# jkulhanek/viewformer

Measured on NVIDIA H100. Metric: novel views/sec (128x128, 9-ctx), higher is better.
Workload: dtype f32 encoder (bit-exact codes) + bf16 transformer/decoder

## Files before the change

### viewformer_b200/csrc/vf_tc_gemm.cu

```cuda
#include "vf_wgmma.cuh"
#include <stdlib.h>

namespace {
using namespace vftc;

constexpr int BLOCK_M = 128;
constexpr int ROW_BYTES = 128;
constexpr int A_STAGE_BYTES = BLOCK_M * ROW_BYTES;
constexpr int NUM_EPI_WARPS = 8;
constexpr int NUM_MMA_THREADS = 32 * NUM_EPI_WARPS;
constexpr int NUM_THREADS = NUM_MMA_THREADS + 128;

struct TcParams {
    CUtensorMap tmA, tmB;
    int conv;
    int M, Ncols;
    int num_k_blocks;
    int batch2;
    int tiles_m, tiles_n, total_tiles;
    int a_bm1, a_bm2, b_bm1, b_bm2;
    int TW, TH, TN, tiles_x, tiles_y, OH, OW, Nimg, cin_blocks, bk_elems;
    int tap_dy[9], tap_dx[9], tap_coff[9];
    int gemm_koff;
    int causal_block, causal_skip_n;
    float alpha;
    const float* bias;
    int bias_mode, act;
    const float* residual;
    float* C_f32;
    __nv_bfloat16* C_bf16;
    long long ldc, c_sb1, c_sb2;
    int vec_ok;
    int halo;
    double* gn_sums;
    int gn_groups, gn_cpg, gn_rows_per_img;
    int exact;
    int exact_kc;
    int exact_clog;
    int exact_kpp;
    int exact_lo_b;
    const float2* norm_mr;
    const float* norm_gamma;
    const float* norm_beta;
    int norm_groups, norm_cpg, norm_swish;
};

constexpr float EXACT_LO_SCALE = 1.0f / 2048.0f;

struct TileInfo {
    int m0, n0, b1, b2, img0, oy0, ox0, nkb;
    bool skip;
};

__device__ __forceinline__ TileInfo decode_tile(const TcParams& p, int t, int block_n) {
    TileInfo ti;
    const int n_tile = t % p.tiles_n;
    const int r = t / p.tiles_n;
    const int m_tile = r % p.tiles_m;
    const int bz = r / p.tiles_m;
    ti.b1 = bz / p.batch2;
    ti.b2 = bz % p.batch2;
    ti.m0 = m_tile * BLOCK_M;
    ti.n0 = n_tile * block_n;
    ti.nkb = p.num_k_blocks;
    ti.skip = false;
    if (p.causal_block > 0) {
        const int lim = ((ti.m0 + BLOCK_M - 1) / p.causal_block + 1) * p.causal_block;
        if (p.causal_skip_n) {
            ti.skip = ti.n0 >= lim;
        } else {
            const int kb = (lim + p.bk_elems - 1) / p.bk_elems;
            if (kb < ti.nkb) ti.nkb = kb;
        }
    }
    ti.img0 = ti.oy0 = ti.ox0 = 0;
    if (p.conv) {
        const int tx = m_tile % p.tiles_x;
        const int q = m_tile / p.tiles_x;
        ti.img0 = (q / p.tiles_y) * p.TN;
        ti.oy0 = (q % p.tiles_y) * p.TH;
        ti.ox0 = tx * p.TW;
    }
    return ti;
}

constexpr int HALO_BYTES = 23552;
__host__ __device__ constexpr int halo_buffers(bool exact) { return exact ? 4 : 2; }
__host__ __device__ constexpr int halo_slots(bool exact) { return exact ? 4 : 6; }
__host__ __device__ constexpr int operand_bytes(int stages, int stage_bytes, int b_stage_bytes, bool exact) {
    return stages * stage_bytes > halo_buffers(exact) * HALO_BYTES + halo_slots(exact) * b_stage_bytes
               ? stages * stage_bytes
               : halo_buffers(exact) * HALO_BYTES + halo_slots(exact) * b_stage_bytes;
}
constexpr int MAX_STAGES = 8;
template <int kBlockN, int kStages, bool kExact>
__host__ __device__ constexpr int tc_smem_bytes() {
    return operand_bytes(kStages, A_STAGE_BYTES + kBlockN * ROW_BYTES, kBlockN * ROW_BYTES, kExact) +
           NUM_EPI_WARPS * 32 * (kBlockN / 2 + 4) * 4  + 1024  + 8 * (2 * MAX_STAGES + 8) ;
}

__device__ __forceinline__ void prefetch_residual_l2(const TcParams& p, const TileInfo& ti, int block_n) {
    const int tw = min(p.TW, p.OW - ti.ox0);
    const uint32_t bytes = (uint32_t)(((long long)(tw - 1) * p.ldc + block_n) * 4);
    for (int r = 0; r < p.TN * p.TH; ++r) {
        const int img = ti.img0 + r / p.TH, oy = ti.oy0 + r % p.TH;
        if (img >= p.Nimg || oy >= p.OH) continue;
        const float* src = p.residual + ((long long)(img * p.OH + oy) * p.OW + ti.ox0) * p.ldc + ti.n0;
        asm volatile("cp.async.bulk.prefetch.L2.global [%0], %1;" ::"l"(src), "r"(bytes) : "memory");
    }
}

__device__ __forceinline__ void normalise_halo(const TcParams& p, uint8_t* tile, int cb, int img, int oy0, int ox0, int tid) {
    const int rows = (p.TW + 2) * (p.TH + 2);
    for (int idx = tid; idx < rows * 8; idx += NUM_MMA_THREADS) {
        const int r = idx >> 3, pc = idx & 7;
        const int py = r / (p.TW + 2), px = r - py * (p.TW + 2);
        const int iy = oy0 - 1 + py, ix = ox0 - 1 + px;
        if (iy < 0 || iy >= p.OH || ix < 0 || ix >= p.OW) continue;
        const int c0 = cb * 64 + ((pc ^ (r & 7)) << 3);
        uint4* ptr = reinterpret_cast<uint4*>(tile + r * ROW_BYTES + pc * 16);
        const uint4 v = *ptr;
        uint32_t w[4] = {v.x, v.y, v.z, v.w};
#pragma unroll
        for (int k = 0; k < 4; ++k) {
            const int c = c0 + 2 * k;
            const float2 ma = __ldg(p.norm_mr + (img * p.norm_groups + c / p.norm_cpg));
            const float2 mb = __ldg(p.norm_mr + (img * p.norm_groups + (c + 1) / p.norm_cpg));
            const float sa = ma.y * __ldg(p.norm_gamma + c), sb = mb.y * __ldg(p.norm_gamma + c + 1);
            float a = __uint_as_float(w[k] << 16), b = __uint_as_float(w[k] & 0xffff0000u);
            a = fmaf(a, sa, __ldg(p.norm_beta + c) - ma.x * sa);
            b = fmaf(b, sb, __ldg(p.norm_beta + c + 1) - mb.x * sb);
            if (p.norm_swish == 1) {
                a = __fdividef(a, 1.0f + __expf(-a));
                b = __fdividef(b, 1.0f + __expf(-b));
            }
            __nv_bfloat162 o = __floats2bfloat162_rn(a, b);
            w[k] = *reinterpret_cast<uint32_t*>(&o);
            if (p.norm_swish == 2) {
                uint32_t h, th;
                asm("mul.rn.bf16x2 %0, %1, %2;" : "=r"(h) : "r"(w[k]), "r"(0x3f003f00u));
                asm("tanh.approx.bf16x2 %0, %1;" : "=r"(th) : "r"(h));
                asm("fma.rn.bf16x2 %0, %1, %2, %1;" : "=r"(w[k]) : "r"(h), "r"(th));
            }
        }
        *ptr = make_uint4(w[0], w[1], w[2], w[3]);
    }
}

template <int kBlockN, int kStages, WgKind kKind>
__global__ void __launch_bounds__(NUM_THREADS, 1) tc_gemm_kernel(const __grid_constant__ TcParams p) {
    constexpr int B_STAGE_BYTES = kBlockN * ROW_BYTES;
    constexpr int STAGE_BYTES = A_STAGE_BYTES + B_STAGE_BYTES;
    constexpr int K_STEPS = 4;
    constexpr int HALF_N = kBlockN / 2;
    constexpr int STG_LD = HALF_N + 4;
    constexpr int STG_BYTES = NUM_EPI_WARPS * 32 * STG_LD * 4;
    constexpr int NACC = kBlockN / 2;
    constexpr bool kExact = kKind == F16;

    extern __shared__ uint8_t smem_raw[];
    uint8_t* smem = reinterpret_cast<uint8_t*>((reinterpret_cast<uintptr_t>(smem_raw) + 1023) & ~(uintptr_t)1023);
    constexpr int OPER_BYTES = operand_bytes(kStages, STAGE_BYTES, B_STAGE_BYTES, kExact);
    float* staging = reinterpret_cast<float*>(smem + OPER_BYTES);
    uint64_t* full_bar = reinterpret_cast<uint64_t*>(smem + OPER_BYTES + STG_BYTES);
    uint64_t* empty_bar = full_bar + MAX_STAGES;
    constexpr int NHB = halo_buffers(kExact);
    uint64_t* a_full_bar = empty_bar + MAX_STAGES;
    uint64_t* a_empty_bar = a_full_bar + NHB;
    constexpr int NG = kStages;
    constexpr int NGH = halo_slots(kExact);
    uint8_t* halo_b_base = smem + NHB * HALO_BYTES;

    const int warp = threadIdx.x >> 5;
    const int lane = threadIdx.x & 31;

    if (threadIdx.x == 0) {
        prefetch_tmap(&p.tmA);
        prefetch_tmap(&p.tmB);
        for (int s = 0; s < MAX_STAGES; ++s) {
            mbar_init(&full_bar[s], 1);
            mbar_init(&empty_bar[s], NUM_MMA_THREADS);
        }
        for (int a = 0; a < NHB; ++a) {
            mbar_init(&a_full_bar[a], 1);
            mbar_init(&a_empty_bar[a], NUM_MMA_THREADS);
        }
        mbar_fence_init();
    }
    __syncthreads();

    if (warp >= NUM_EPI_WARPS) {
        setmaxnreg_dec<40>();
        if (warp == NUM_EPI_WARPS && elect_one()) {
            int stage = 0;
            uint32_t phase = 0;
            int ab = 0;
            uint32_t aphase = 0, tpar = 0;
            for (int t = blockIdx.x; t < p.total_tiles; t += gridDim.x, tpar ^= 1) {
                const TileInfo ti = decode_tile(p, t, kBlockN);
                if (ti.skip) continue;
                const uint32_t halo_bytes = (uint32_t)((p.TW + 2) * (p.TH + 2)) * ROW_BYTES;
                if (kExact && p.halo) {
                    auto load_halves = [&](int h) {
                        for (int cb = 0; cb < p.cin_blocks; ++cb) {
                            const int hb = 2 * h + cb;
                            mbar_wait(&a_empty_bar[hb], tpar ^ 1, "vf_tc_gemm producer(halo)");
                            mbar_expect_tx(&a_full_bar[hb], halo_bytes);
                            tma_load_4d(smem + hb * HALO_BYTES, &p.tmA, &a_full_bar[hb], (h ? 0 : p.exact_clog) + cb * p.bk_elems,
                                        ti.ox0 - 1, ti.oy0 - 1, ti.img0);
                        }
                    };
                    load_halves(0);
                    if (p.residual && p.vec_ok && ti.n0 + kBlockN <= p.Ncols) prefetch_residual_l2(p, ti, kBlockN);
                    int j = 0, tap = 0, cb = 0;
                    for (int kb = 0; kb < ti.nkb; ++kb) {
                        if (kb == NGH) load_halves(1);
                        mbar_wait(&empty_bar[stage], phase ^ 1, "vf_tc_gemm producer");
                        mbar_expect_tx(&full_bar[stage], (uint32_t)B_STAGE_BYTES);
                        tma_load_4d(halo_b_base + stage * B_STAGE_BYTES, &p.tmB, &full_bar[stage],
                                    ((tap * 2 + (j == 1 ? 1 : 0)) * p.cin_blocks + cb) * p.bk_elems, ti.n0, 0, 0);
                        if (++cb == p.cin_blocks) { cb = 0; if (++tap == 9) { tap = 0; ++j; } }
                        if (++stage == NGH) { stage = 0; phase ^= 1; }
                    }
                    continue;
                }
                if (p.halo) {
                    const int nkb = 9 * p.cin_blocks;
                    int tap = 0, cb = 0;
                    for (int kb = 0; kb < nkb; ++kb) {
                        mbar_wait(&empty_bar[stage], phase ^ 1, "vf_tc_gemm producer");
                        mbar_expect_tx(&full_bar[stage], (uint32_t)B_STAGE_BYTES);
                        if (tap == 0) {
                            mbar_wait(&a_empty_bar[ab], aphase ^ 1, "vf_tc_gemm producer(halo)");
                            mbar_expect_tx(&a_full_bar[ab], halo_bytes);
                            tma_load_4d(smem + ab * HALO_BYTES, &p.tmA, &a_full_bar[ab], cb * p.bk_elems, ti.ox0 - 1, ti.oy0 - 1, ti.img0);
                            if (++ab == 2) { ab = 0; aphase ^= 1; }
                        }
                        tma_load_4d(halo_b_base + stage * B_STAGE_BYTES, &p.tmB, &full_bar[stage], (tap * p.cin_blocks + cb) * p.bk_elems,
                                    ti.n0, 0, 0);
                        if (++tap == 9) { tap = 0; ++cb; }
                        if (++stage == NGH) { stage = 0; phase ^= 1; }
                    }
                    continue;
                }
                if (kExact && p.conv && p.residual && p.vec_ok && ti.n0 + kBlockN <= p.Ncols) prefetch_residual_l2(p, ti, kBlockN);
                for (int kb = 0; kb < ti.nkb; ++kb) {
                    mbar_wait(&empty_bar[stage], phase ^ 1, "vf_tc_gemm producer");
                    mbar_expect_tx(&full_bar[stage], (uint32_t)STAGE_BYTES);
                    uint8_t* sa = smem + stage * STAGE_BYTES;
                    uint8_t* sb = sa + A_STAGE_BYTES;
                    int kcoord_b = kb * p.bk_elems;
                    if (p.conv) {
                        int kbr = kb, a_half = 0;
                        if (p.exact) {
                            const int j = kb / p.exact_kpp;
                            kbr = kb - j * p.exact_kpp;
                            a_half = (j == 0) ? p.exact_clog : 0;
                            const int tap_ = kbr / p.cin_blocks, cb_ = kbr - tap_ * p.cin_blocks;
                            kcoord_b = ((tap_ * 2 + (j == 1 ? 1 : 0)) * p.cin_blocks + cb_) * p.bk_elems;
                        }
                        const int tap = kbr / p.cin_blocks;
                        const int cb = kbr - tap * p.cin_blocks;
                        tma_load_4d(sa, &p.tmA, &full_bar[stage], a_half + p.tap_coff[tap] + cb * p.bk_elems, ti.ox0 + p.tap_dx[tap],
                                    ti.oy0 + p.tap_dy[tap], ti.img0);
                    } else {
                        int kcoord_a = kb * p.bk_elems;
                        if (p.exact) {
                            const int j = kb / p.exact_kpp, kbr = kb - j * p.exact_kpp;
                            kcoord_a = (j == 0 ? p.exact_clog : 0) + kbr * p.bk_elems;
                            kcoord_b = (j == 1 ? p.exact_lo_b : 0) + kbr * p.bk_elems;
                        }
                        if (p.gemm_koff) kcoord_a += p.tap_coff[ti.b1];
                        tma_load_4d(sa, &p.tmA, &full_bar[stage], kcoord_a, ti.m0, ti.b2 * p.a_bm2, ti.b1 * p.a_bm1);
                    }
                    tma_load_4d(sb, &p.tmB, &full_bar[stage], kcoord_b, ti.n0, ti.b2 * p.b_bm2, ti.b1 * p.b_bm1);
                    if (++stage == NG) { stage = 0; phase ^= 1; }
                }
            }
        }
        return;
    }

    setmaxnreg_inc<232>();
    const int wg = warp >> 2;
    const int quarter = warp & 3;
    const int col_half = warp >> 2;
    float* stg = staging + warp * (32 * STG_LD);
    int stage = 0, ab = 0;
    uint32_t phase = 0, aphase = 0, tpar = 0;

    const bool col_split = kExact && p.halo && p.TW == 16;
    auto to_staging = [&](const float (&v)[NACC], float sc) {
        const int r_lo = 64 * wg + 16 * (warp & 3) + (lane >> 2);
#pragma unroll
        for (int j = 0; j < NACC / 4; ++j) {
#pragma unroll
            for (int h = 0; h < 2; ++h) {
                const int r = col_split ? 16 * (2 * (warp & 3) + h) + 8 * wg + (lane >> 2) : r_lo + 8 * h;
                const int c = 8 * j + 2 * (lane & 3);
                float* dst = staging + ((c / HALF_N) * 4 + (r >> 5)) * (32 * STG_LD) + (r & 31) * STG_LD + (c % HALF_N);
                *reinterpret_cast<float2*>(dst) = make_float2(v[4 * j + 2 * h] * sc, v[4 * j + 2 * h + 1] * sc);
            }
        }
    };

    for (int t = blockIdx.x; t < p.total_tiles; t += gridDim.x, tpar ^= 1) {
        const TileInfo ti = decode_tile(p, t, kBlockN);
        if (ti.skip) continue;

        float acc[NACC];
        float csum[kExact ? NACC : 1];
        auto k_loop = [&]() {
            const int nkb = (p.halo && !kExact) ? 9 * p.cin_blocks : ti.nkb;
            const int nsmall = p.exact ? 2 * p.exact_kpp / p.exact_kc : 0;
            int prev_stage = -1, prev_halo = -1, in_chunk = 0, ck = 0, tap = 0, j = 0, cb = 0;
            bool fresh = true;
            uint32_t a_base = 0;
            const uint32_t pitch = (uint32_t)(p.TW + 2);
            const uint32_t wg_rows = p.TW == 16 ? 8u : 8u * pitch;
            auto retire_prev = [&]() {
                if (prev_stage >= 0) mbar_arrive(&empty_bar[prev_stage]);
                if (prev_halo >= 0) mbar_arrive(&a_empty_bar[prev_halo]);
                prev_stage = prev_halo = -1;
            };
#pragma unroll 1
            for (int kb = 0; kb < nkb; ++kb) {
                uint64_t adesc, bdesc;
                int this_halo = (p.halo && tap == 8) ? ab : -1;
                if (kExact && p.halo) {
                    const int hb = (j == 0 ? 0 : 2) + cb;
                    if (tap == 0 && j < 2) mbar_wait(&a_full_bar[hb], tpar, "vf_tc_gemm mma(halo)");
                    this_halo = (tap == 8 && j != 1) ? hb : -1;
                    mbar_wait(&full_bar[stage], phase, "vf_tc_gemm mma");
                    const uint32_t a_addr = smem_u32(smem + hb * HALO_BYTES) +
                                            ((uint32_t)(tap / 3) * pitch + (uint32_t)(tap % 3) + (uint32_t)wg * wg_rows) * ROW_BYTES;
                    adesc = sw128_desc(a_addr, pitch * ROW_BYTES);
                    bdesc = sw128_desc(smem_u32(halo_b_base + stage * B_STAGE_BYTES));
                } else if (p.halo) {
                    if (tap == 0) {
                        mbar_wait(&a_full_bar[ab], aphase, "vf_tc_gemm mma(halo)");
                        a_base = smem_u32(smem + ab * HALO_BYTES);
                        if (!kExact && p.norm_mr) {
                            normalise_halo(p, smem + ab * HALO_BYTES, kb / 9, ti.img0, ti.oy0, ti.ox0, threadIdx.x);
                            fence_async_smem();
                            named_sync(1, NUM_MMA_THREADS);
                        }
                    }
                    mbar_wait(&full_bar[stage], phase, "vf_tc_gemm mma");
                    const uint32_t a_addr = a_base + ((uint32_t)(tap / 3) * pitch + (uint32_t)(tap % 3) + (uint32_t)(8 * wg) * pitch) * ROW_BYTES;
                    adesc = sw128_desc(a_addr, pitch * ROW_BYTES);
                    bdesc = sw128_desc(smem_u32(halo_b_base + stage * B_STAGE_BYTES));
                } else {
                    mbar_wait(&full_bar[stage], phase, "vf_tc_gemm mma");
                    const uint32_t sa = smem_u32(smem + stage * STAGE_BYTES);
                    adesc = sw128_desc(sa + (uint32_t)(wg * 64 * ROW_BYTES));
                    bdesc = sw128_desc(sa + A_STAGE_BYTES);
                }
                wgmma_fence();
#pragma unroll
                for (int k = 0; k < K_STEPS; ++k)
                    wgmma_ss<kBlockN, kKind>(acc, adesc + (uint64_t)(2 * k), bdesc + (uint64_t)(2 * k), (fresh && k == 0) ? 0u : 1u);
                wgmma_commit();
                fresh = false;
                wgmma_wait<1>();
                retire_prev();
                prev_stage = stage;
                prev_halo = this_halo;
                if (kExact && p.halo) {
                    if (++stage == NGH) { stage = 0; phase ^= 1; }
                    if (++cb == p.cin_blocks) { cb = 0; if (++tap == 9) { tap = 0; ++j; } }
                } else if (p.halo) {
                    if (++stage == NGH) { stage = 0; phase ^= 1; }
                    if (++tap == 9) { tap = 0; if (++ab == 2) { ab = 0; aphase ^= 1; } }
                } else {
                    if (++stage == NG) { stage = 0; phase ^= 1; }
                }
                if (kExact && ++in_chunk == p.exact_kc) {
                    in_chunk = 0;
                    wgmma_wait<0>();
                    reg_fence(acc);
                    const float sc = (ck < nsmall ? EXACT_LO_SCALE : 1.0f) * p.alpha;
                    if (ck == 0) {
#pragma unroll
                        for (int i = 0; i < NACC; ++i) csum[i] = acc[i] * sc;
                    } else {
#pragma unroll
                        for (int i = 0; i < NACC; ++i) csum[i] = fmaf(acc[i], sc, csum[i]);
                    }
                    ++ck;
                    fresh = true;
                }
            }
            wgmma_wait<0>();
            reg_fence(acc);
            retire_prev();
        };
        if constexpr (kExact) k_loop();

        const int row = quarter * 32 + lane;
        long long my_off;
        int my_ok, gm;
        if (p.conv) {
            const int lx = row % p.TW;
            const int q = row / p.TW;
            const int ly = q % p.TH;
            const int ln = q / p.TH;
            const int img = ti.img0 + ln, oy = ti.oy0 + ly, ox = ti.ox0 + lx;
            my_ok = (img < p.Nimg) && (oy < p.OH) && (ox < p.OW);
            gm = (img * p.OH + oy) * p.OW + ox;
            my_off = (long long)gm * p.ldc;
        } else {
            gm = ti.m0 + row;
            my_ok = gm < p.M;
            my_off = (long long)ti.b1 * p.c_sb1 + (long long)ti.b2 * p.c_sb2 + (long long)gm * p.ldc;
        }
        const float bias_m = (p.bias_mode == VF_BIAS_M && my_ok) ? __ldg(p.bias + gm) : 0.f;

        constexpr int VPR = HALF_N / 4;
        constexpr int RPI = 32 / VPR;
        constexpr int ITERS = 32 / RPI;
        const int r_sub = lane / VPR;
        const int c_ln = (lane % VPR) * 4;
        const int n_ln = ti.n0 + col_half * HALF_N + c_ln;
        const bool fast = p.vec_ok && (ti.n0 + kBlockN <= p.Ncols);
        auto residual_at = [&](int i) {
            const int rr = i * RPI + r_sub;
            const int ok = __shfl_sync(0xffffffffu, my_ok, rr);
            const long long off_row = __shfl_sync(0xffffffffu, my_off, rr);
            const long long o = ok ? off_row + n_ln : (long long)n_ln;
            return __ldg(reinterpret_cast<const float4*>(p.residual + o));
        };
        constexpr int RB = kExact ? ITERS / 2 : ITERS;
        float4 resv[RB];
        auto load_residual = [&](int i0) {
            if (fast && p.residual) {
#pragma unroll
                for (int i = 0; i < RB; ++i) resv[i] = residual_at(i0 + i);
            }
        };
        if constexpr (!kExact) load_residual(0);
        float4 bias4 = make_float4(0.f, 0.f, 0.f, 0.f);
        if (fast && p.bias_mode == VF_BIAS_N) bias4 = __ldg(reinterpret_cast<const float4*>(p.bias + n_ln));

        if constexpr (!kExact) k_loop();
        named_sync(1, NUM_MMA_THREADS);
        if constexpr (kExact) to_staging(csum, 1.0f);
        else to_staging(acc, p.alpha);
        named_sync(1, NUM_MMA_THREADS);

        if (fast) {
            float gs = 0.f, gq = 0.f;
#pragma unroll
            for (int i = 0; i < ITERS; ++i) {
                if (kExact && i % RB == 0) load_residual(i);
                const int rr = i * RPI + r_sub;
                const int ok = __shfl_sync(0xffffffffu, my_ok, rr);
                const long long off_row = __shfl_sync(0xffffffffu, my_off, rr);
                const float bm = __shfl_sync(0xffffffffu, bias_m, rr);
                float4 v = *reinterpret_cast<const float4*>(stg + rr * STG_LD + c_ln);
                if (p.bias_mode == VF_BIAS_N) { v.x += bias4.x; v.y += bias4.y; v.z += bias4.z; v.w += bias4.w; }
                else { v.x += bm; v.y += bm; v.z += bm; v.w += bm; }
                if (p.act == VF_ACT_GELU_ERF) { v.x = vf_gelu_erf(v.x); v.y = vf_gelu_erf(v.y); v.z = vf_gelu_erf(v.z); v.w = vf_gelu_erf(v.w); }
                if (p.residual) {
                    const float4 r = resv[i % RB];
                    v.x += r.x; v.y += r.y; v.z += r.z; v.w += r.w;
                }
                if (ok) {
                    gs += (v.x + v.y) + (v.z + v.w);
                    gq += (v.x * v.x + v.y * v.y) + (v.z * v.z + v.w * v.w);
                    const long long off = off_row + n_ln;
                    if (p.C_f32) *reinterpret_cast<float4*>(p.C_f32 + off) = v;
                    if (p.C_bf16) {
                        __nv_bfloat162 lo = __floats2bfloat162_rn(v.x, v.y), hi = __floats2bfloat162_rn(v.z, v.w);
                        uint2 u;
                        u.x = *reinterpret_cast<uint32_t*>(&lo);
                        u.y = *reinterpret_cast<uint32_t*>(&hi);
                        *reinterpret_cast<uint2*>(p.C_bf16 + off) = u;
                    }
                }
            }
            if (p.gn_sums) {
                const unsigned okmask = __ballot_sync(0xffffffffu, my_ok);
#pragma unroll
                for (int o = VPR; o < 32; o <<= 1) {
                    gs += __shfl_xor_sync(0xffffffffu, gs, o);
                    gq += __shfl_xor_sync(0xffffffffu, gq, o);
                }
                const int lpg = p.gn_cpg >> 2;
                for (int o = 1; o < lpg; o <<= 1) {
                    gs += __shfl_xor_sync(0xffffffffu, gs, o);
                    gq += __shfl_xor_sync(0xffffffffu, gq, o);
                }
                const int gm_first = __shfl_sync(0xffffffffu, gm, okmask ? (__ffs(okmask) - 1) : 0);
                if (okmask && r_sub == 0 && (lane % lpg) == 0) {
                    const long long slot = ((long long)(gm_first / p.gn_rows_per_img) * p.gn_groups + n_ln / p.gn_cpg) * 2;
                    atomicAdd(p.gn_sums + slot, (double)gs);
                    atomicAdd(p.gn_sums + slot + 1, (double)gq);
                }
            }
        } else {
#pragma unroll 1
            for (int rr = 0; rr < 32; ++rr) {
                const int ok = __shfl_sync(0xffffffffu, my_ok, rr);
                const long long off_row = __shfl_sync(0xffffffffu, my_off, rr);
                const float bm = __shfl_sync(0xffffffffu, bias_m, rr);
                if (!ok) continue;
                for (int c = lane; c < HALF_N; c += 32) {
                    const int n = ti.n0 + col_half * HALF_N + c;
                    if (n >= p.Ncols) continue;
                    float x = stg[rr * STG_LD + c];
                    x += (p.bias_mode == VF_BIAS_N) ? __ldg(p.bias + n) : bm;
                    if (p.act == VF_ACT_GELU_ERF) x = vf_gelu_erf(x);
                    const long long off = off_row + n;
                    if (p.residual) x += __ldg(p.residual + off);
                    if (p.C_f32) p.C_f32[off] = x;
                    if (p.C_bf16) p.C_bf16[off] = __float2bfloat16(x);
                }
            }
        }
    }
}

int make_tmap(CUtensorMap* tm, int dtype, const void* base, const uint64_t dims[4], const uint64_t strides_bytes[3],
              const uint32_t box[4]) {
    EncodeTiledFn fn = encode_fn();
    if (!fn) { vf_set_error("vf_tc_gemm: cuTensorMapEncodeTiled unavailable"); return VF_ERR_CUDA; }
    cuuint64_t gdim[4] = {dims[0], dims[1], dims[2], dims[3]};
    cuuint64_t gstr[3] = {strides_bytes[0], strides_bytes[1], strides_bytes[2]};
    cuuint32_t bx[4] = {box[0], box[1], box[2], box[3]};
    cuuint32_t es[4] = {1, 1, 1, 1};
    CUresult r = fn(tm, dtype == VF_BF16 ? CU_TENSOR_MAP_DATA_TYPE_BFLOAT16 : CU_TENSOR_MAP_DATA_TYPE_FLOAT32, 4,
                    const_cast<void*>(base), gdim, gstr, bx, es, CU_TENSOR_MAP_INTERLEAVE_NONE, CU_TENSOR_MAP_SWIZZLE_128B,
                    CU_TENSOR_MAP_L2_PROMOTION_L2_256B, CU_TENSOR_MAP_FLOAT_OOB_FILL_NONE);
    if (r != CUDA_SUCCESS) {
        vf_set_error("vf_tc_gemm: cuTensorMapEncodeTiled failed (%d): dims=[%llu,%llu,%llu,%llu] strides=[%llu,%llu,%llu] box=[%u,%u,%u,%u]",
                     (int)r, (unsigned long long)dims[0], (unsigned long long)dims[1], (unsigned long long)dims[2],
                     (unsigned long long)dims[3], (unsigned long long)strides_bytes[0], (unsigned long long)strides_bytes[1],
                     (unsigned long long)strides_bytes[2], box[0], box[1], box[2], box[3]);
        return VF_ERR_CUDA;
    }
    return VF_OK;
}

template <int kBlockN, int kStages, WgKind kKind>
int launch(const TcParams& prm, dim3 grid, cudaStream_t st) {
    constexpr int smem = tc_smem_bytes<kBlockN, kStages, kKind == F16>();
    static_assert(kStages <= MAX_STAGES, "ring depth");
    static_assert(smem <= 232448, "shared memory budget");
    static vf_per_device_flag configured_pd;
    bool& configured = configured_pd.current();
    if (!configured) {
        cudaError_t e = cudaFuncSetAttribute(tc_gemm_kernel<kBlockN, kStages, kKind>, cudaFuncAttributeMaxDynamicSharedMemorySize, smem);
        if (e != cudaSuccess) { vf_set_error("vf_tc_gemm: cudaFuncSetAttribute: %s", cudaGetErrorString(e)); return VF_ERR_CUDA; }
        configured = true;
    }
    tc_gemm_kernel<kBlockN, kStages, kKind><<<grid, NUM_THREADS, smem, st>>>(prm);
    VF_CHECK_LAUNCH("vf_tc_gemm");
    return VF_OK;
}

template <int kBlockN, int kStages>
int launch_kind(const TcParams& prm, WgKind kind, dim3 grid, cudaStream_t st) {
    if (kind == TF32) return launch<kBlockN, kStages, TF32>(prm, grid, st);
    if (kind == F16) return launch<kBlockN, kStages, F16>(prm, grid, st);
    return launch<kBlockN, kStages, BF16>(prm, grid, st);
}

}

extern "C" int vf_tc_gemm(const vf_tc_gemm_t* q, vf_stream_t s) {
    VF_CHECK_ARG(q && q->A && q->B, "vf_tc_gemm: null operand");
    VF_CHECK_ARG(q->C_f32 || q->C_bf16, "vf_tc_gemm: no output");
    VF_CHECK_ARG(q->ab_dtype == VF_BF16 || q->ab_dtype == VF_F32 || q->ab_dtype == VF_F16X2, "vf_tc_gemm: bad dtype");
    const bool exact = q->ab_dtype == VF_F16X2;
    if (exact) {
        VF_CHECK_ARG(q->C_f32 && !q->C_bf16 && !q->norm_mean_rstd && q->causal_block == 0,
                     "vf_tc_gemm: VF_F16X2 (exact split-fp16) operands need an fp32 output and no causal / fused-norm options");
        if (q->conv) VF_CHECK_ARG(q->Ctot % 2 == 0 && q->alpha == 1.0f, "vf_tc_gemm: exact conv needs [hi | lo] channels and alpha = 1");
        else VF_CHECK_ARG(q->K % 64 == 0 && q->exact_lo_a >= q->K && q->exact_lo_b >= q->K && q->exact_lo_a % 8 == 0 && q->exact_lo_b % 8 == 0,
                          "vf_tc_gemm: exact GEMM needs K %% 64 == 0 and lo-half offsets >= K (K=%d lo_a=%lld lo_b=%lld)", q->K,
                          (long long)q->exact_lo_a, (long long)q->exact_lo_b);
    }
    VF_CHECK_ARG(q->bias_mode == VF_BIAS_NONE || q->bias, "vf_tc_gemm: bias pointer missing");
    VF_CHECK_ARG(!q->norm_mean_rstd || q->conv, "vf_tc_gemm: fused input GroupNorm is a convolution option");
    const bool tf32 = q->ab_dtype == VF_F32;
    const int tm_dtype = tf32 ? VF_F32 : VF_BF16;
    const int es = tf32 ? 4 : 2;
    const int bk = ROW_BYTES / es;

    TcParams prm;
    memset(&prm, 0, sizeof(prm));
    prm.conv = q->conv;
    prm.Ncols = q->Ncols;
    prm.bk_elems = bk;
    prm.alpha = q->alpha;
    prm.bias = q->bias;
    prm.bias_mode = q->bias_mode;
    prm.act = q->act;
    prm.residual = q->residual;
    prm.C_f32 = q->C_f32;
    prm.C_bf16 = reinterpret_cast<__nv_bfloat16*>(q->C_bf16);
    prm.ldc = q->ldc;
    prm.causal_block = q->causal_block;
    prm.causal_skip_n = q->causal_skip_n;

    const int block_n = (q->Ncols > 64) ? 128 : 64;
    const int b_box_rows = block_n;
    dim3 grid;
    int rc;
    if (q->conv) {
        VF_CHECK_ARG(q->ntaps >= 1 && q->ntaps <= 9, "vf_tc_gemm: ntaps");
        VF_CHECK_ARG(q->Cin % bk == 0 && q->Ctot % (16 / es) == 0, "vf_tc_gemm: conv Cin=%d must be a multiple of %d", q->Cin, bk);
        VF_CHECK_ARG(q->causal_block == 0, "vf_tc_gemm: causal with conv");
        int TW = q->OW >= 16 ? 16 : (q->OW >= 8 ? 8 : (q->OW >= 4 ? 4 : (q->OW >= 2 ? 2 : 1)));
        int TH = 128 / TW;
        if (TH > q->OH) { TH = 1; while (TH * 2 <= q->OH) TH *= 2; }
        int TN = 128 / (TW * TH);
        bool halo = q->ntaps == 9 && q->OH == q->H && q->OW == q->W &&
                    (exact ? q->Ctot == 2 * q->Cin && q->Cin <= 2 * bk && TN == 1 && TW >= 8
                           : q->Ctot == q->Cin && q->OH >= 16 && q->OW >= 8);
        for (int t = 0; halo && t < 9; ++t) halo = q->tap_dy[t] == t / 3 - 1 && q->tap_dx[t] == t % 3 - 1 && q->tap_coff[t] == 0;
        if (halo && !exact) { TW = 8; TH = 16; TN = 1; }
        prm.halo = halo ? 1 : 0;
        if (q->norm_mean_rstd) {
            VF_CHECK_ARG(halo && q->ab_dtype == VF_BF16 && q->H >= 32 && q->Ncols % 128 == 0 && q->Cin % 64 == 0,
                         "vf_tc_gemm: fused input GroupNorm needs a 3x3 stride-1 bf16 conv on a map >= 32 rows (Cin %% 64 == 0, Cout %% 128 == 0)");
            VF_CHECK_ARG(q->norm_gamma && q->norm_beta && q->norm_groups > 0 && q->Cin % q->norm_groups == 0,
                         "vf_tc_gemm: fused input GroupNorm needs gamma, beta and a group count dividing Cin");
            prm.norm_mr = reinterpret_cast<const float2*>(q->norm_mean_rstd);
            prm.norm_gamma = q->norm_gamma;
            prm.norm_beta = q->norm_beta;
            prm.norm_groups = q->norm_groups;
            prm.norm_cpg = q->Cin / q->norm_groups;
            prm.norm_swish = q->norm_swish;
        }
        VF_CHECK_ARG(TW * TH * TN == 128 && TN <= 256, "vf_tc_gemm: cannot tile %dx%d output", q->OH, q->OW);
        prm.TW = TW; prm.TH = TH; prm.TN = TN;
        prm.tiles_x = (q->OW + TW - 1) / TW;
        prm.tiles_y = (q->OH + TH - 1) / TH;
        prm.OH = q->OH; prm.OW = q->OW; prm.Nimg = q->N;
        prm.cin_blocks = q->Cin / bk;
        prm.num_k_blocks = q->ntaps * prm.cin_blocks;
        if (exact) {
            prm.exact = 1;
            prm.exact_kpp = prm.num_k_blocks;
            prm.exact_clog = q->Ctot / 2;
            prm.exact_kc = (prm.num_k_blocks % 3 == 0) ? 3 : 1;
            prm.num_k_blocks *= 3;
        }
        prm.M = q->N * q->OH * q->OW;
        prm.batch2 = 1;
        for (int t = 0; t < q->ntaps; ++t) { prm.tap_dy[t] = q->tap_dy[t]; prm.tap_dx[t] = q->tap_dx[t]; prm.tap_coff[t] = q->tap_coff[t]; }
        const uint64_t dimsA[4] = {(uint64_t)q->Ctot, (uint64_t)q->W, (uint64_t)q->H, (uint64_t)q->N};
        const uint64_t strA[3] = {(uint64_t)q->Ctot * es, (uint64_t)q->W * q->Ctot * es, (uint64_t)q->H * q->W * q->Ctot * es};
        const uint32_t boxA[4] = {(uint32_t)bk, (uint32_t)(halo ? TW + 2 : TW), (uint32_t)(halo ? TH + 2 : TH), (uint32_t)TN};
        if ((rc = make_tmap(&prm.tmA, tm_dtype, q->A, dimsA, strA, boxA)) != VF_OK) return rc;
        const uint64_t Ktot = (uint64_t)q->ntaps * q->Cin * (exact ? 2 : 1);
        const uint64_t dimsB[4] = {Ktot, (uint64_t)q->Ncols, 1, 1};
        const uint64_t strB[3] = {Ktot * es, Ktot * es * q->Ncols, Ktot * es * q->Ncols};
        const uint32_t boxB[4] = {(uint32_t)bk, (uint32_t)b_box_rows, 1, 1};
        if ((rc = make_tmap(&prm.tmB, tm_dtype, q->B, dimsB, strB, boxB)) != VF_OK) return rc;
        const int ntiles_img = (q->N + TN - 1) / TN;
        grid = dim3(prm.tiles_x * prm.tiles_y * ntiles_img, (q->Ncols + block_n - 1) / block_n, 1);
    } else {
        VF_CHECK_ARG(q->M > 0 && q->Ncols > 0 && q->K > 0 && q->batch1 > 0 && q->batch2 > 0, "vf_tc_gemm: bad shape");
        VF_CHECK_ARG((q->lda * es) % 16 == 0 && (q->ldb * es) % 16 == 0, "vf_tc_gemm: row strides must be 16-byte multiples");
        VF_CHECK_ARG((q->a_sb1 * es) % 16 == 0 && (q->a_sb2 * es) % 16 == 0 && (q->b_sb1 * es) % 16 == 0 && (q->b_sb2 * es) % 16 == 0,
                     "vf_tc_gemm: batch strides must be 16-byte multiples");
        prm.M = q->M;
        prm.batch2 = q->batch2;
        prm.num_k_blocks = (q->K + bk - 1) / bk;
        if (exact) {
            prm.exact = 1;
            prm.exact_kpp = prm.num_k_blocks;
            prm.exact_clog = (int)q->exact_lo_a;
            prm.exact_lo_b = (int)q->exact_lo_b;
            prm.exact_kc = prm.exact_kpp % 4 == 0 ? 4 : (prm.exact_kpp % 3 == 0 ? 3 : (prm.exact_kpp % 2 == 0 ? 2 : 1));
            prm.num_k_blocks *= 3;
        }
        prm.c_sb1 = q->c_sb1; prm.c_sb2 = q->c_sb2;
        long long max_koff = 0;
        if (q->ntaps > 0) {
            VF_CHECK_ARG(q->ntaps == q->batch1 && q->ntaps <= 9, "vf_tc_gemm: gemm K offsets need ntaps == batch1 <= 9");
            prm.gemm_koff = 1;
            for (int t = 0; t < q->ntaps; ++t) {
                VF_CHECK_ARG(q->tap_coff[t] >= 0 && q->tap_coff[t] % 8 == 0, "vf_tc_gemm: K offsets must be non-negative multiples of 8 (16-byte TMA box starts)");
                prm.tap_coff[t] = q->tap_coff[t];
                if (q->tap_coff[t] > max_koff) max_koff = q->tap_coff[t];
            }
        }
        prm.a_bm1 = (q->batch1 > 1 && q->a_sb1 != 0) ? 1 : 0;
        prm.a_bm2 = (q->batch2 > 1 && q->a_sb2 != 0) ? 1 : 0;
        prm.b_bm1 = (q->batch1 > 1 && q->b_sb1 != 0) ? 1 : 0;
        prm.b_bm2 = (q->batch2 > 1 && q->b_sb2 != 0) ? 1 : 0;
        const uint64_t fbA = (uint64_t)q->lda * es * (uint64_t)q->M, fbB = (uint64_t)q->ldb * es * (uint64_t)q->Ncols;
        const uint64_t dimsA[4] = {(uint64_t)((exact ? q->exact_lo_a + q->K : q->K) + max_koff), (uint64_t)q->M, prm.a_bm2 ? (uint64_t)q->batch2 : 1, prm.a_bm1 ? (uint64_t)q->batch1 : 1};
        const uint64_t strA[3] = {(uint64_t)q->lda * es, prm.a_bm2 ? (uint64_t)q->a_sb2 * es : fbA, prm.a_bm1 ? (uint64_t)q->a_sb1 * es : fbA};
        const uint32_t boxA[4] = {(uint32_t)bk, (uint32_t)BLOCK_M, 1, 1};
        if ((rc = make_tmap(&prm.tmA, tm_dtype, q->A, dimsA, strA, boxA)) != VF_OK) return rc;
        const uint64_t dimsB[4] = {(uint64_t)(exact ? q->exact_lo_b + q->K : q->K), (uint64_t)q->Ncols, prm.b_bm2 ? (uint64_t)q->batch2 : 1, prm.b_bm1 ? (uint64_t)q->batch1 : 1};
        const uint64_t strB[3] = {(uint64_t)q->ldb * es, prm.b_bm2 ? (uint64_t)q->b_sb2 * es : fbB, prm.b_bm1 ? (uint64_t)q->b_sb1 * es : fbB};
        const uint32_t boxB[4] = {(uint32_t)bk, (uint32_t)b_box_rows, 1, 1};
        if ((rc = make_tmap(&prm.tmB, tm_dtype, q->B, dimsB, strB, boxB)) != VF_OK) return rc;
        VF_CHECK_ARG(q->causal_block == 0 || (q->causal_block % bk == 0 || bk % q->causal_block == 0), "vf_tc_gemm: causal block");
        grid = dim3((q->M + BLOCK_M - 1) / BLOCK_M, (q->Ncols + block_n - 1) / block_n, q->batch1 * q->batch2);
    }
    prm.tiles_m = (int)grid.x;
    prm.tiles_n = (int)grid.y;
    const long long total = (long long)prm.tiles_m * grid.y * grid.z;
    VF_CHECK_ARG(total > 0 && total < (1ll << 31), "vf_tc_gemm: tile count out of range");
    prm.total_tiles = (int)total;
    static int num_sms = 0;
    if (num_sms == 0) {
        int dev = 0;
        cudaGetDevice(&dev);
        if (cudaDeviceGetAttribute(&num_sms, cudaDevAttrMultiProcessorCount, dev) != cudaSuccess || num_sms <= 0) num_sms = 132;
    }
    const dim3 pgrid((unsigned)(total < num_sms ? total : num_sms), 1, 1);
    {
        auto a16 = [](const void* p) { return (reinterpret_cast<uintptr_t>(p) & 15) == 0; };
        auto a8 = [](const void* p) { return (reinterpret_cast<uintptr_t>(p) & 7) == 0; };
        prm.vec_ok = (q->ldc % 4 == 0) && (q->c_sb1 % 4 == 0) && (q->c_sb2 % 4 == 0) && a16(q->C_f32) && a8(q->C_bf16) && a16(q->residual) &&
                     a16(q->bias);
    }
    if (q->gn_sums) {
        const int C = q->Ncols;
        VF_CHECK_ARG(q->gn_groups > 0 && C % q->gn_groups == 0, "vf_tc_gemm: gn_groups");
        const int cpg = C / q->gn_groups;
        const long long rpi = q->conv ? (long long)q->OH * q->OW : q->gn_rows_per_img;
        const long long rows = q->conv ? (long long)q->N * q->OH * q->OW : (long long)q->M;
        VF_CHECK_ARG(cpg % 4 == 0 && cpg <= 32 && 32 % cpg == 0 && C % block_n == 0 && prm.vec_ok && rpi >= 32 && rpi % 32 == 0 &&
                         rows % rpi == 0 && (q->conv ? (prm.TW * prm.TH) % 32 == 0 : q->batch1 * q->batch2 == 1),
                     "vf_tc_gemm: fused GroupNorm statistics unsupported for this shape (C=%d groups=%d rows/img=%lld)", C, q->gn_groups, rpi);
        prm.gn_sums = q->gn_sums;
        prm.gn_groups = q->gn_groups;
        prm.gn_cpg = cpg;
        prm.gn_rows_per_img = (int)rpi;
        cudaError_t e = cudaMemsetAsync(q->gn_sums, 0, sizeof(double) * 2 * q->gn_groups * (rows / rpi), vf_s(s));
        if (e != cudaSuccess) { vf_set_error("vf_tc_gemm: memset gn_sums: %s", cudaGetErrorString(e)); return VF_ERR_CUDA; }
    }
    cudaStream_t st = vf_s(s);
    const WgKind kind = tf32 ? TF32 : (exact ? F16 : BF16);
    if (block_n == 128) return launch_kind<128, 4>(prm, kind, pgrid, st);
    return launch_kind<64, 6>(prm, kind, pgrid, st);
}
```

Before: 318.4.

## Double-buffer exact-mode accumulators to overlap chunk folding with next WGMMA

```diff
diff --git a/viewformer_b200/csrc/vf_tc_gemm.cu b/viewformer_b200/csrc/vf_tc_gemm.cu
--- a/viewformer_b200/csrc/vf_tc_gemm.cu
+++ b/viewformer_b200/csrc/vf_tc_gemm.cu
@@ -309,12 +309,11 @@
         if (ti.skip) continue;
 
         float acc[NACC];
+        float acc_b[kExact ? NACC : 1];
         float csum[kExact ? NACC : 1];
         auto k_loop = [&]() {
             const int nkb = (p.halo && !kExact) ? 9 * p.cin_blocks : ti.nkb;
-            const int nsmall = p.exact ? 2 * p.exact_kpp / p.exact_kc : 0;
-            int prev_stage = -1, prev_halo = -1, in_chunk = 0, ck = 0, tap = 0, j = 0, cb = 0;
-            bool fresh = true;
+            int prev_stage = -1, prev_halo = -1, tap = 0, j = 0, cb = 0;
             uint32_t a_base = 0;
             const uint32_t pitch = (uint32_t)(p.TW + 2);
             const uint32_t wg_rows = p.TW == 16 ? 8u : 8u * pitch;
@@ -323,8 +322,7 @@
                 if (prev_halo >= 0) mbar_arrive(&a_empty_bar[prev_halo]);
                 prev_stage = prev_halo = -1;
             };
-#pragma unroll 1
-            for (int kb = 0; kb < nkb; ++kb) {
+            auto k_step = [&](float (&a)[NACC], int kb, bool fresh) {
                 uint64_t adesc, bdesc;
                 int this_halo = (p.halo && tap == 8) ? ab : -1;
                 if (kExact && p.halo) {
@@ -359,9 +357,8 @@
                 wgmma_fence();
 #pragma unroll
                 for (int k = 0; k < K_STEPS; ++k)
-                    wgmma_ss<kBlockN, kKind>(acc, adesc + (uint64_t)(2 * k), bdesc + (uint64_t)(2 * k), (fresh && k == 0) ? 0u : 1u);
+                    wgmma_ss<kBlockN, kKind>(a, adesc + (uint64_t)(2 * k), bdesc + (uint64_t)(2 * k), (fresh && k == 0) ? 0u : 1u);
                 wgmma_commit();
-                fresh = false;
                 wgmma_wait<1>();
                 retire_prev();
                 prev_stage = stage;
@@ -375,24 +372,47 @@
                 } else {
                     if (++stage == NG) { stage = 0; phase ^= 1; }
                 }
-                if (kExact && ++in_chunk == p.exact_kc) {
-                    in_chunk = 0;
-                    wgmma_wait<0>();
-                    reg_fence(acc);
+            };
+            if constexpr (kExact) {
+                const int nch = nkb / p.exact_kc;
+                const int nsmall = 2 * p.exact_kpp / p.exact_kc;
+                enum { NO_FOLD, FOLD_FIRST, FOLD };
+                auto fold = [&](float (&a)[NACC], int ck, bool first) {
+                    reg_fence(a);
                     const float sc = (ck < nsmall ? EXACT_LO_SCALE : 1.0f) * p.alpha;
-                    if (ck == 0) {
-#pragma unroll
-                        for (int i = 0; i < NACC; ++i) csum[i] = acc[i] * sc;
+                    if (first) {
+#pragma unroll
+                        for (int i = 0; i < NACC; ++i) csum[i] = a[i] * sc;
                     } else {
 #pragma unroll
-                        for (int i = 0; i < NACC; ++i) csum[i] = fmaf(acc[i], sc, csum[i]);
+                        for (int i = 0; i < NACC; ++i) csum[i] = fmaf(a[i], sc, csum[i]);
                     }
-                    ++ck;
-                    fresh = true;
-                }
-            }
-            wgmma_wait<0>();
-            reg_fence(acc);
+                };
+                auto chunk = [&](float (&a)[NACC], float (&prev)[NACC], int ck, int fold_prev) {
+                    k_step(a, ck * p.exact_kc, true);
+                    if (fold_prev != NO_FOLD) fold(prev, ck - 1, fold_prev == FOLD_FIRST);
+#pragma unroll 1
+                    for (int i = 1; i < p.exact_kc; ++i) k_step(a, ck * p.exact_kc + i, false);
+                };
+                chunk(acc, acc_b, 0, NO_FOLD);
+                chunk(acc_b, acc, 1, FOLD_FIRST);
+#pragma unroll 1
+                for (int ck = 2;; ck += 2) {
+                    chunk(acc, acc_b, ck, FOLD);
+                    if (ck + 1 == nch) { wgmma_wait<0>(); fold(acc, ck, false); break; }
+                    chunk(acc_b, acc, ck + 1, FOLD);
+                    if (ck + 2 == nch) { wgmma_wait<0>(); fold(acc_b, ck + 1, false); break; }
+                }
+            } else {
+                bool fresh = true;
+#pragma unroll 1
+                for (int kb = 0; kb < nkb; ++kb) {
+                    k_step(acc, kb, fresh);
+                    fresh = false;
+                }
+                wgmma_wait<0>();
+                reg_fence(acc);
+            }
             retire_prev();
         };
         if constexpr (kExact) k_loop();
@@ -432,6 +452,10 @@
         };
         constexpr int RB = kExact ? ITERS / 2 : ITERS;
         float4 resv[RB];
+        if constexpr (kExact) {
+#pragma unroll
+            for (int i = 0; i < RB; ++i) resv[i] = make_float4(0.f, 0.f, 0.f, 0.f);
+        }
         auto load_residual = [&](int i0) {
             if (fast && p.residual) {
 #pragma unroll
```

New measurement: 321.1, median of 6. Within noise of the previous version (+0.8%).
